# singer-yang/Aberration-Aware-Depth-from-Focus

Measured on NVIDIA B200. Metric: focal-stack Mpix*slices/s (fused PSFNet+PSF render), higher is better.
Workload: dtype fp16 hi/lo split, 3 terms for L1-L7, 2 terms on calibrated fp16 weights for L8, L9 and the head (worst case over any image 7.5e-5), f32 accumulate

## Files before the change

aberration-aware-depth-from-focus_b200/csrc/aadff_api.cu:

```cuda
#include <cuda_fp16.h>
#include <cuda_runtime.h>

#include <atomic>
#include <cmath>
#include <cstdio>
#include <cstring>
#include <mutex>
#include <string>
#include <vector>

#include "../../include/aadff.h"
#include "fused_tc_kernel.cuh"
#include "fused_fast2_kernel.cuh"
#include "gather_kernel.cuh"
#include "gather_coalesced_kernel.cuh"
#include "gather_strip_kernel.cuh"
#include "mlp_fp32_kernel.cuh"
#include "thinlens_kernel.cuh"
#include "focus_kernel.cuh"
#include "psf_conv_kernel.cuh"
#include "train_kernels.cuh"
#include "preprocess_kernel.cuh"
#include "spline_rotate_kernel.cuh"
#include "econ_calib.h"
// ... 432 lines not shown
        for (int l = 1; l < n_layers - 1; ++l, ++gi) {
            TcGroup& g = h->groups[gi];
            g.w_off = (uint32_t)(pack.size() * sizeof(__half));
            g.K = (uint16_t)dims[l];
            g.N = TC_HID;
            g.terms = 3;
            g.bias_off = (uint16_t)bias_tc.size();
            g.new_a = 1;
            g.tap0 = 0;
            pack_bias_slab(biases[l], TC_HID, pack);
            pack_group(weights[l], dims[l + 1], dims[l], 0, TC_HID, pack);
            bias_tc.insert(bias_tc.end(), biases[l], biases[l] + TC_HID);
        }
        h->n_hidden = gi;
        const int L = n_layers - 1;
        const int head_bias0 = (int)bias_tc.size();
        h->head_bias0 = head_bias0;
        bias_tc.resize(head_bias0 + nh_pad, 0.f);
        for (int n = 0; n < h->kk; ++n) bias_tc[head_bias0 + n] = -1.4426950408889634f * biases[L][n];
        for (int b = 0; b < n_head_blocks; ++b, ++gi) {
            TcGroup& g = h->groups[gi];
            const int N = std::min(256, nh_pad - 256 * b);
            g.w_off = (uint32_t)(pack.size() * sizeof(__half));
            g.K = TC_HID;
            g.N = (uint16_t)N;
            g.terms = 3;
            g.bias_off = (uint16_t)(head_bias0 + 256 * b);
            g.new_a = (b == 0);
            g.tap0 = (uint16_t)(256 * b);
            pack_group(weights[L], h->kk, TC_HID, 256 * b, N, pack);
        }
        h->n_groups = gi;
        h->n_bias = (int)bias_tc.size();
        h->host_dims.assign(dims, dims + n_layers + 1);
        for (int l = 0; l < n_layers; ++l) {
            h->host_w.emplace_back(weights[l], weights[l] + (size_t)dims[l] * dims[l + 1]);
            h->host_b.emplace_back(biases[l], biases[l] + dims[l + 1]);
        }
        h->pack_bytes = pack.size() * sizeof(__half);
        std::vector<float> w0b0(320);
        std::memcpy(w0b0.data(), weights[0], 256 * sizeof(float));
        std::memcpy(w0b0.data() + 256, biases[0], 64 * sizeof(float));
        __half* dp = nullptr;
        int rc = upload(pack, &dp);
        if (rc) { aadff_psfnet_destroy(h); return rc; }
        h->d_wpack = reinterpret_cast<uint8_t*>(dp);
        rc = upload(bias_tc, &h->d_bias_tc);
        if (rc) { aadff_psfnet_destroy(h); return rc; }
        rc = upload(w0b0, &h->d_w0b0);
        if (rc) { aadff_psfnet_destroy(h); return rc; }
        const int so = h->smem_optin;
        const auto attr = cudaFuncAttributeMaxDynamicSharedMemorySize;
        CREATE_TRY(cudaFuncSetAttribute(fused_psfnet_render_kernel<true, false, 0>, attr, so));
#define AADFF_SET_ATTR(U)                                                                        \
        CREATE_TRY(cudaFuncSetAttribute(fused_psfnet_render_kernel<false, false, U>, attr, so));   \
        CREATE_TRY(cudaFuncSetAttribute(fused_psfnet_render_kernel<false, false, U, true>, attr, so));   \
        CREATE_TRY(cudaFuncSetAttribute(fused_psfnet_render_kernel<false, true, U>, attr, so));
        AADFF_SET_ATTR(0) AADFF_SET_ATTR(1) AADFF_SET_ATTR(3) AADFF_SET_ATTR(13) AADFF_SET_ATTR(12) AADFF_SET_ATTR(15)
#undef AADFF_SET_ATTR
        CREATE_TRY(cudaFuncSetAttribute(fused_psfnet_render_kernel<false, false, 14>, attr, so));
        CREATE_TRY(cudaFuncSetAttribute(fused_psfnet_render_kernel<false, true, 14>, attr, so));
    }
#undef CREATE_TRY
    *out = h;
    return AADFF_OK;
}

int aadff_psfnet_destroy(aadff_psfnet_t h) {
    if (!h) return AADFF_OK;
    DeviceGuard guard(h->device);
    for (float* p : h->owned) cudaFree(p);
    cudaFree(h->d_wpack);
    cudaFree(h->d_wpack_econ);
    cudaFree(h->d_bias_tc);
    cudaFree(h->d_w0b0);
    cudaFree(h->ws);
    if (h->ws_stream) cudaStreamDestroy(h->ws_stream);
    if (h->ws_copy_stream) cudaStreamDestroy(h->ws_copy_stream);
    for (cudaEvent_t e : h->ws_events) cudaEventDestroy(e);
    delete h;
    return AADFF_OK;
}

static int ensure_econ(aadff_psfnet_t h) {
    std::lock_guard<std::mutex> lock(h->econ_mu);
    if (h->econ_ready) return AADFF_OK;
    const int n_layers = h->n_layers, L = n_layers - 1;
    std::vector<const float*> W(n_layers), B(n_layers);
    for (int l = 0; l < n_layers; ++l) { W[l] = h->host_w[l].data(); B[l] = h->host_b[l].data(); }
    std::vector<std::vector<float>> wq;
    calibrate_econ(W.data(), B.data(), h->host_dims.data(), n_layers, TC_ECON_FIRST_LAYER, wq);
    std::vector<__half> pack;
    for (int g2 = 0; g2 < h->n_groups; ++g2) {
        const bool hidden = g2 < h->n_hidden;
        const int l = hidden ? g2 + 1 : L;
        h->w_off_econ[g2] = h->groups[g2].w_off;
        if (l < TC_ECON_FIRST_LAYER || wq[l].empty()) continue;
        h->w_off_econ[g2] = (uint32_t)(h->pack_bytes + pack.size() * sizeof(__half));
        if (hidden) {
            pack_bias_slab(B[l], TC_HID, pack);
            pack_group(wq[l].data(), h->host_dims[l + 1], h->host_dims[l], 0, TC_HID, pack);
        } else {
            pack_group(wq[l].data(), h->kk, TC_HID, h->groups[g2].tap0, h->groups[g2].N, pack);
        }
    }
    uint8_t* d = nullptr;
    CUDA_TRY(cudaMalloc(reinterpret_cast<void**>(&d), h->pack_bytes + pack.size() * sizeof(__half)));
    cudaError_t e = cudaMemcpy(d, h->d_wpack, h->pack_bytes, cudaMemcpyDeviceToDevice);
    if (e == cudaSuccess) e = cudaMemcpy(d + h->pack_bytes, pack.data(), pack.size() * sizeof(__half), cudaMemcpyHostToDevice);
    if (e != cudaSuccess) {
        cudaFree(d);
        return fail(AADFF_E_CUDA, std::string("econ weight upload: ") + cudaGetErrorString(e));
    }
    h->d_wpack_econ = d;
// ... 89 lines not shown
        P.n_tiles = (tile_row1 - tile_row0) * P.tiles_x;
        if (P.n_tiles <= 0) return AADFF_OK;
    }
    if (probes != nullptr) {
        P.probes = probes;
        P.psf_out = psf_out;
        P.n_probes = n_probes;
        P.n_tiles = (n_probes + TC_M - 1) / TC_M;
    }
    P.trace = g_trace.load();
    P.dbg = (uint32_t)g_dbg_flags.load();
    uint32_t halo_bytes = (uint32_t)(TC_TILE_H + ra.ks - 1) * TC_HALO_PITCH * 16;
    if (probes != nullptr) halo_bytes = std::max<uint32_t>(halo_bytes, 8 * 32 * 9 * 4);
    const uint32_t bias_bytes = (uint32_t)(h->n_bias - h->head_bias0) * 4;
    const uint32_t ones_bytes = 2 * TC_A_LBO;
    const uint32_t bslab_bytes = 2 * TC_BSLAB_BYTES;
    const uint32_t fixed = 2 * TC_A_PART_BYTES + bias_bytes + 320 * 4 + halo_bytes + TC_M * 5 * 4 + TC_BAR_BYTES + ones_bytes +
                           bslab_bytes + 16;
    int stages = 4;
    while (stages >= 2 && fixed + (uint32_t)stages * TC_STAGE_BYTES > (uint32_t)h->smem_optin) --stages;
    if (stages < 2) return fail(AADFF_E_UNSUPPORTED, "shared memory budget exceeded for this kernel size / channel count");
    bool any_lo = false;
    for (int i = 0; i < h->n_groups; ++i) any_lo |= (P.g[i].terms >= 2);
    P.off_stage = 2 * TC_A_PART_BYTES;
    P.off_bias = P.off_stage + stages * TC_STAGE_BYTES;
    P.off_w0 = P.off_bias + bias_bytes;
    P.off_halo = P.off_w0 + 320 * 4;
    P.off_red = P.off_halo + halo_bytes;
    P.off_bar = P.off_red + TC_M * 5 * 4;
    P.off_ones = (P.off_bar + TC_BAR_BYTES + 15u) & ~15u;
    P.off_bslab = P.off_ones + ones_bytes;
    const uint32_t smem = P.off_bslab + bslab_bytes;
    P.kslab = (!any_lo && stages == 4) ? 2 : 1;
    P.n_stages = (P.kslab == 2) ? 4 : stages;
    int grid = (int)std::min<long long>(P.n_tiles, h->num_sms);
    bool all3 = true, all1 = true, econ_pat = true, econ8_pat = true, mixed_pat = true, aligned = (P.n_stages == 4 && P.kslab == 1);
    for (int i = 0; i < h->n_groups; ++i) {
        const int t = P.g[i].terms;
        all3 &= (t == 3);
        all1 &= (t == 1);
        econ_pat &= (t == (i < TC_ECON_FIRST_GROUP ? 3 : 2));
        econ8_pat &= (t == (i < TC_ECON8_FIRST_GROUP ? 3 : 2));
        mixed_pat &= (t == (i < TC_MIXED_FIRST_GROUP ? 3 : 1));
        aligned &= (((P.g[i].K / TC_SLAB_K) * (t == 3 ? 2 : 1)) % 4 == 0);
    }
    static_assert(TC_ECON_FIRST_GROUP == TC_ECON_FIRST_LAYER - 1, "group g holds layer g + 1");
    int uni = 0;
    if (all3 && P.kslab == 1) uni = aligned ? 13 : 3;
    else if (all1 && P.kslab == 2) uni = 1;
    else if (econ_pat && aligned) uni = 12;
    else if (econ8_pat && aligned && h->n_groups > TC_ECON8_FIRST_GROUP) uni = 14;
    else if (mixed_pat && aligned) uni = 15;
    const bool cl2 = P.probes == nullptr && P.trace == nullptr && uni != 0 && uni != 14 && (P.dbg & 8u) && h->num_sms >= 2;
    if (cl2) {
        grid = (int)std::min<long long>((P.n_tiles + 1) & ~1ll, (long long)(h->num_sms & ~1));
        cudaLaunchConfig_t cfg{};
        cfg.gridDim = dim3((unsigned)grid);
        cfg.blockDim = dim3(TC_NT);
        cfg.dynamicSmemBytes = smem;
        cfg.stream = st;
        cudaLaunchAttribute la[1];
        la[0].id = cudaLaunchAttributeClusterDimension;
        la[0].val.clusterDim.x = 2; la[0].val.clusterDim.y = 1; la[0].val.clusterDim.z = 1;
        cfg.attrs = la;
        cfg.numAttrs = 1;
        cudaError_t le = cudaSuccess;
        switch (uni) {
            case 1: le = cudaLaunchKernelEx(&cfg, fused_psfnet_render_kernel<false, false, 1, true>, P); break;
            case 3: le = cudaLaunchKernelEx(&cfg, fused_psfnet_render_kernel<false, false, 3, true>, P); break;
            case 13: le = cudaLaunchKernelEx(&cfg, fused_psfnet_render_kernel<false, false, 13, true>, P); break;
            case 12: le = cudaLaunchKernelEx(&cfg, fused_psfnet_render_kernel<false, false, 12, true>, P); break;
            default: le = cudaLaunchKernelEx(&cfg, fused_psfnet_render_kernel<false, false, 15, true>, P); break;
        }
        if (le != cudaSuccess) return fail(AADFF_E_CUDA, std::string("cluster launch: ") + cudaGetErrorString(le));
    } else if (P.trace != nullptr && P.probes == nullptr) {
        fused_psfnet_render_kernel<true, false, 0><<<grid, TC_NT, smem, st>>>(P);
    } else {
#define AADFF_LAUNCH(U)                                                                                   \
        case U:                                                                                           \
            if (P.probes != nullptr) fused_psfnet_render_kernel<false, true, U><<<grid, TC_NT, smem, st>>>(P);   \
            else fused_psfnet_render_kernel<false, false, U><<<grid, TC_NT, smem, st>>>(P);               \
            break;
        switch (uni) {
            AADFF_LAUNCH(1) AADFF_LAUNCH(3) AADFF_LAUNCH(13) AADFF_LAUNCH(12) AADFF_LAUNCH(14) AADFF_LAUNCH(15)
            default:
                if (P.probes != nullptr) fused_psfnet_render_kernel<false, true, 0><<<grid, TC_NT, smem, st>>>(P);
                else fused_psfnet_render_kernel<false, false, 0><<<grid, TC_NT, smem, st>>>(P);
        }
#undef AADFF_LAUNCH
    }
    g_launches.fetch_add(1);
    CUDA_TRY(cudaGetLastError());
    return AADFF_OK;
}

static int render_stack_impl(aadff_psfnet_t h, const float* img, const float* depth, const float* foc, int foc_stride,
                             float* out, const int64_t out_strides[5], int N, int C, int S, int H, int W, float d_min,
                             float d_max, int mode, void* stream, long long tile_row0 = 0, long long tile_row1 = -1);

int aadff_tile_row_height(void) { return TC_TILE_H; }
int aadff_econ_first_group(void) { return TC_ECON_FIRST_GROUP; }

int aadff_render_stack_rows_f32(aadff_psfnet_t h, const float* img, const float* depth, const float* foc, float* out,
                                const int64_t out_strides[5], int N, int C, int S, int H, int W, float d_min,
                                float d_max, int mode, int64_t tile_row_begin, int64_t tile_row_end, void* stream) {
    const long long total = (long long)N * S * ((H + TC_TILE_H - 1) / TC_TILE_H);
    if (tile_row_begin < 0 || tile_row_end < tile_row_begin || tile_row_end > total)
        return fail(AADFF_E_INVALID, "tile-row range outside [0, N*S*ceil(H/8)]");
    return render_stack_impl(h, img, depth, foc, S, out, out_strides, N, C, S, H, W, d_min, d_max, mode, stream,
                             tile_row_begin, tile_row_end);
}

int aadff_render_stack_f32(aadff_psfnet_t h, const float* img, const float* depth, const float* foc, float* out,
                           const int64_t out_strides[5], int N, int C, int S, int H, int W, float d_min,
                           float d_max, int mode, void* stream) {
    return render_stack_impl(h, img, depth, foc, S, out, out_strides, N, C, S, H, W, d_min, d_max, mode, stream);
}

static int render_stack_impl(aadff_psfnet_t h, const float* img, const float* depth, const float* foc, int foc_stride,
                             float* out, const int64_t out_strides[5], int N, int C, int S, int H, int W, float d_min,
                             float d_max, int mode, void* stream, long long tile_row0, long long tile_row1) {
    if (!h || !img || !depth || !foc || !out || !out_strides) return fail(AADFF_E_INVALID, "null argument");
    if (N < 0 || C < 1 || S < 1 || H < 1 || W < 1) return fail(AADFF_E_INVALID, "bad shape");
    if (mode < 0 || mode > 5) return fail(AADFF_E_INVALID, "unknown mode");
    if (d_max == d_min) return fail(AADFF_E_INVALID, "d_max == d_min");
    if (N == 0) return AADFF_OK;
    DeviceGuard guard(h->device);
    if (!guard.ok) return fail(AADFF_E_CUDA, "cannot select device");
    cudaStream_t st = static_cast<cudaStream_t>(stream);
    RenderArgs ra{};
    ra.img = img; ra.depth = depth; ra.foc = foc; ra.out = out;
    ra.os_n = out_strides[0]; ra.os_c = out_strides[1]; ra.os_s = out_strides[2];
    ra.os_h = out_strides[3]; ra.os_w = out_strides[4];
    ra.N = N; ra.S = S; ra.H = H; ra.W = W; ra.ks = h->ks; ra.Ctot = C;
    ra.foc_stride = foc_stride;
    ra.d_min = d_min;
    ra.d_range = d_max - d_min;
    ra.step_x = (W > 1) ? (1.0f - (-1.0f)) / (float)(W - 1) : 0.f;
    ra.step_y = (H > 1) ? (-1.0f - 1.0f) / (float)(H - 1) : 0.f;
    for (int c0 = 0; c0 < C; c0 += 4) {
        ra.c0 = c0;
        ra.C = std::min(4, C - c0);
// ... 544 lines not shown
```

aberration-aware-depth-from-focus_b200/csrc/fused_tc_kernel.cuh:

```cuda
#pragma once
#include <cuda_fp16.h>
#include <cuda_runtime.h>
#include "ptx_sm100.cuh"
#include "render_args.h"

namespace aadff {

constexpr int TC_TILE_H = 8;
constexpr int TC_TILE_W = 16;
constexpr int TC_M = TC_TILE_H * TC_TILE_W;
constexpr int TC_HALO_PITCH = 48;
constexpr int TC_HID = 256;
constexpr int TC_SLAB_K = 32;
constexpr int TC_STAGE_BYTES = TC_HID * TC_SLAB_K * 2;
constexpr int TC_A_PART_BYTES = TC_M * TC_HID * 2;
constexpr int TC_A_LBO = TC_M * 16;
constexpr int TC_EPI_WARPS = 8;
constexpr int TC_EPI_THREADS = TC_EPI_WARPS * 32;
constexpr int TC_NT = 64 + TC_EPI_THREADS;
constexpr int TC_MAX_GROUPS = 16;
constexpr int TC_MAX_STAGES = 8;
constexpr int TC_MAX_KS = 31;
constexpr int TC_MAX_C = 4;
constexpr int TC_BAR_BYTES = 256;
// ... 65 lines not shown
__device__ __forceinline__ uint32_t pack_half2_relu(float a, float b) {
    uint32_t r;
    asm("cvt.rn.relu.f16x2.f32 %0, %1, %2;" : "=r"(r) : "f"(b), "f"(a));
    return r;
}

__device__ __forceinline__ uint32_t pack_half2_relu_rz(float a, float b) {
    uint32_t r;
    asm("cvt.rz.relu.f16x2.f32 %0, %1, %2;" : "=r"(r) : "f"(b), "f"(a));
    return r;
}

__device__ __forceinline__ void store_split8(const float (&v)[8], uint32_t addr_hi, uint32_t addr_lo, bool need_lo) {
    uint32_t h[4];
#pragma unroll
    for (int u = 0; u < 4; ++u) h[u] = pack_half2(v[2 * u], v[2 * u + 1]);
    st_shared_v4(addr_hi, h[0], h[1], h[2], h[3]);
    if (need_lo) {
        uint32_t l[4];
#pragma unroll
        for (int u = 0; u < 4; ++u) {
            const float2 f = __half22float2(*reinterpret_cast<__half2*>(&h[u]));
            l[u] = pack_half2(v[2 * u] - f.x, v[2 * u + 1] - f.y);
        }
        st_shared_v4(addr_lo, l[0], l[1], l[2], l[3]);
    }
}

__device__ __forceinline__ void epi_group8(const uint32_t* acc, uint32_t a_hi, uint32_t a_lo,
                                           uint32_t kg, uint32_t a_row, bool need_lo) {
    if (!need_lo) {
        uint32_t h[4];
#pragma unroll
        for (int u = 0; u < 4; ++u) h[u] = pack_half2_relu(__uint_as_float(acc[2 * u]), __uint_as_float(acc[2 * u + 1]));
        st_shared_v4(a_hi + kg * TC_A_LBO + a_row, h[0], h[1], h[2], h[3]);
        return;
    }
    uint32_t h[4], l[4];
#pragma unroll
    for (int u = 0; u < 4; ++u) {
        const float a0 = __uint_as_float(acc[2 * u]), a1 = __uint_as_float(acc[2 * u + 1]);
        h[u] = pack_half2_relu_rz(a0, a1);
        const float2 f = __half22float2(*reinterpret_cast<__half2*>(&h[u]));
        l[u] = pack_half2_relu(a0 - f.x, a1 - f.y);
    }
    const uint32_t off = kg * TC_A_LBO + a_row;
    st_shared_v4(a_hi + off, h[0], h[1], h[2], h[3]);
    st_shared_v4(a_lo + off, l[0], l[1], l[2], l[3]);
}

constexpr int TC_WARP_PRODUCER = TC_EPI_WARPS;
constexpr int TC_WARP_MMA = TC_EPI_WARPS + 1;

template <bool TRACE, bool PRED, int UNI, bool CL2 = false>
__global__ void __launch_bounds__(TC_NT, 1) fused_psfnet_render_kernel(const __grid_constant__ TcParams P) {
    static_assert(!(CL2 && (PRED || TRACE)), "the cluster variant exists for the render kernels only");
    constexpr int UM = UNI % 10;
    const uint32_t cta_rank = CL2 ? cluster_ctarank() : 0u;
    const long long first_tile = CL2 ? (long long)(blockIdx.x & ~1u) : (long long)blockIdx.x;
    const long long my_iters = (P.n_tiles > first_tile) ? (P.n_tiles - first_tile + gridDim.x - 1) / gridDim.x : 0;
    constexpr bool ALIGNED = UNI >= 10;
    const int kslab_c = (UM == 3 || UM == 2 || UM == 4 || UM == 5) ? 1 : UM == 1 ? 2 : P.kslab;
    auto terms_of = [&](int gi) -> int {
        return UM == 3 ? 3 : UM == 1 ? 1 : UM == 2 ? (gi < TC_ECON_FIRST_GROUP ? 3 : 2)
                                         : UM == 4 ? (gi < TC_ECON8_FIRST_GROUP ? 3 : 2)
                                         : UM == 5 ? (gi < TC_MIXED_FIRST_GROUP ? 3 : 1) : (int)P.g[gi].terms;
    };
    extern __shared__ __align__(1024) uint8_t smem[];
    const uint32_t sbase = smem_u32(smem);
    const int warp = threadIdx.x >> 5, lane = threadIdx.x & 31;
    const RenderArgs& ra = P.ra;

    const uint32_t a_hi = sbase, a_lo = sbase + TC_A_PART_BYTES;
    const uint32_t stage0 = sbase + P.off_stage;
    const int stage_bytes = kslab_c * TC_STAGE_BYTES, stages_in_area = 4 / kslab_c;
    auto stage_addr = [&](int st) {
        return st < stages_in_area ? stage0 + st * stage_bytes : a_lo + (st - stages_in_area) * stage_bytes;
    };
    float* s_bias = reinterpret_cast<float*>(smem + P.off_bias);
    float* s_w0 = reinterpret_cast<float*>(smem + P.off_w0);
    float4* s_halo = reinterpret_cast<float4*>(smem + P.off_halo);
    float* s_red = reinterpret_cast<float*>(smem + P.off_red);
    const uint32_t bar0 = sbase + P.off_bar;
    auto bar_full = [&](int s) { return bar0 + 8u * s; };
    auto bar_empty = [&](int s) { return bar0 + 8u * (TC_MAX_STAGES + s); };
    auto bar_aready = [&](int j) { return bar0 + 8u * (2 * TC_MAX_STAGES + j); };
    auto bar_accfull = [&](int b) { return bar0 + 8u * (2 * TC_MAX_STAGES + 8 + b); };
    auto bar_accfree = [&](int b) { return bar0 + 8u * (2 * TC_MAX_STAGES + 10 + b); };
    auto bar_bfull = [&]() { return bar0 + 8u * (2 * TC_MAX_STAGES + 12); };
    auto bar_bempty = [&]() { return bar0 + 8u * (2 * TC_MAX_STAGES + 13); };
    volatile uint32_t* tmem_slot = reinterpret_cast<volatile uint32_t*>(smem + P.off_bar + 8 * (2 * TC_MAX_STAGES + 14));
    static_assert(8 * (2 * TC_MAX_STAGES + 14) + 4 <= TC_BAR_BYTES, "barrier area too small");

    if (threadIdx.x == 0) {
        for (int s = 0; s < TC_MAX_STAGES; ++s) { mbar_init(bar_full(s), 1); mbar_init(bar_empty(s), CL2 ? 2 : 1); }
        for (int j = 0; j < 8; ++j)
            mbar_init(bar_aready(j), (kslab_c == 2 || j < 4) ? TC_EPI_WARPS : 2 * TC_EPI_WARPS);
        for (int b = 0; b < 2; ++b) { mbar_init(bar_accfull(b), 1); mbar_init(bar_accfree(b), TC_EPI_WARPS); }
        mbar_init(bar_bfull(), 1);
        mbar_init(bar_bempty(), 1);
        fence_mbar_init();
    }
    for (int i = threadIdx.x; i < P.n_bias - P.bias_skip; i += TC_NT) s_bias[i] = __ldg(P.bias + P.bias_skip + i);
    for (int i = threadIdx.x; i < 2 * TC_M; i += TC_NT) {
        uint4 v = make_uint4(0u, 0u, 0u, 0u);
        if (i < TC_M) v.x = 0x3C003C00u;
        *reinterpret_cast<uint4*>(smem + P.off_ones + (i < TC_M ? 0 : TC_A_LBO) + (i % TC_M) * 16) = v;
    }
    for (int i = threadIdx.x; i < TC_BSLAB_BYTES / 16; i += TC_NT)
// ... 248 lines not shown
                if constexpr (PRED) {
                    const long long m = tile * TC_M + row;
                    nx_in = (m < P.n_probes) ? __ldg(reinterpret_cast<const float4*>(P.probes) + m)
                                             : make_float4(0.f, 0.f, 0.f, 0.f);
                } else {
                    int n, s, h0, w0;
                    tile_coords(tile, n, s, h0, w0);
                    const int hc = min(h0 + ty, ra.H - 1), wc = min(w0 + tx, ra.W - 1);
                    d = __ldg(ra.depth + ((long long)n * ra.H + hc) * ra.W + wc);
                    f = __ldg(ra.foc + (long long)n * ra.foc_stride + s);
                }
            }
        };
        float nx_depth = 0.f, nx_foc = 0.f;
        fetch_dz(blockIdx.x, nx_depth, nx_foc);

        auto layer0 = [&](long long t) {
            float x, y, z, fz;
            if constexpr (PRED) {
                x = nx_in.x; y = nx_in.y; z = nx_in.z; fz = nx_in.w;
            } else {
                int n, s, h0, w0;
                tile_coords(t, n, s, h0, w0);
                x = coord_x(min(w0 + tx, ra.W - 1), ra.W, ra.step_x);
                y = coord_y(min(h0 + ty, ra.H - 1), ra.H, ra.step_y);
                z = depth_to_z(nx_depth, ra.d_min, ra.d_range);
                fz = depth_to_z(nx_foc, ra.d_min, ra.d_range);
            }
            const bool need_lo = terms_of(0) >= 2;
#pragma unroll
            for (int i = 0; i < 4; ++i) {
                const int kg = fine ? ((i >> 1) * 4 + 2 * hh + (i & 1)) : (hh * 4 + i);
                float v[8];
#pragma unroll
                for (int u = 0; u < 8; ++u) {
                    const int f = kg * 8 + u;
                    const float4 wv = *reinterpret_cast<const float4*>(s_w0 + f * 4);
                    float a = s_w0[256 + f];
                    a = fmaf(wv.x, x, a); a = fmaf(wv.y, y, a); a = fmaf(wv.z, z, a); a = fmaf(wv.w, fz, a);
                    v[u] = fmaxf(a, 0.f);
                }
                const uint32_t off = (uint32_t)kg * TC_A_LBO + a_row;
                store_split8(v, a_hi + off, a_lo + off, need_lo);
            }
            fence_proxy_async_smem();
            __syncwarp();
            if (lane == 0) {
                if (fine) { mbar_arrive(bar_aready(0)); mbar_arrive(bar_aready(1)); }
                else mbar_arrive(bar_aready(0));
            }
        };
        if (my_iters > 0) layer0(blockIdx.x);

        long long tile = blockIdx.x;
        for (long long iter = 0; iter < my_iters; ++iter, tile += gridDim.x) {
            const bool dummy = CL2 && tile >= P.n_tiles;
            int n = 0, s = 0, h0 = 0, w0 = 0;
            if constexpr (!PRED) tile_coords(dummy ? 0 : tile, n, s, h0, w0);
            const int h = h0 + ty, w = w0 + tx;
            const long long m_row = tile * TC_M + row;
            const bool valid = PRED ? (m_row < P.n_probes) : ((h < ra.H) && (w < ra.W) && !dummy);
            tr.ev(0x800);
            fetch_dz(tile + gridDim.x, nx_depth, nx_foc);

            named_bar_sync(1, TC_EPI_THREADS);
            const float* img_n = ra.img + ((long long)n * ra.Ctot + ra.c0) * ra.H * ra.W;
            const long long cstride = (long long)ra.H * ra.W;
            auto halo_fetch = [&](int idx, float4& v) -> int {
                if (PRED || dummy || idx >= HH * HW) return -1;
                const int yy = idx / HW, xx = idx - yy * HW;
                const int gy = min(max(h0 + yy - r, 0), ra.H - 1), gx = min(max(w0 + xx - r, 0), ra.W - 1);
                const float* px = img_n + (long long)gy * ra.W + gx;
                v.x = __ldg(px);
                v.y = ra.C > 1 ? __ldg(px + cstride) : 0.f;
                v.z = ra.C > 2 ? __ldg(px + 2 * cstride) : 0.f;
                v.w = ra.C > 3 ? __ldg(px + 3 * cstride) : 0.f;
                return yy * TC_HALO_PITCH + xx;
            };

            for (int gi = 0; gi < P.n_hidden; ++gi) {
                const int buf = (int)(gcount & 1);
                float4 hv = make_float4(0.f, 0.f, 0.f, 0.f);
                const int hslot = halo_fetch(gi * TC_EPI_THREADS + et, hv);
                tr.ev(0xA00 + gi);
                mbar_wait(bar_accfull(buf), (afphase >> buf) & 1);
                afphase ^= 1u << buf;
                tc_fence_after_sync();
                tr.ev(0xB00 + gi);
                const bool need_lo = terms_of(gi + 1) >= 2;
                const uint32_t t_acc = t_lane + buf * 256;
                uint32_t rr[2][32], rf[2][16];
                if (fine) {
                    tmem_ld16(t_acc + hh * 16, rf[0]);
                    tmem_ld16(t_acc + 32 + hh * 16, rf[1]);
                } else {
                    tmem_ld32(t_acc + hh * 32, rr[0]);
                }
#pragma unroll
                for (int j = 0; j < 4; ++j) {
                    tmem_ld_wait();
                    if (j < 3) tmem_ld32(t_acc + (j + 1) * 64 + hh * 32, rr[(j + 1) & 1]);
                    if (j == 0 && fine) {
#pragma unroll
                        for (int c = 0; c < 2; ++c) {
                            const int col = c * 32 + hh * 16;
#pragma unroll
                            for (int i = 0; i < 2; ++i)
                                epi_group8(&rf[c][i * 8], a_hi, a_lo, col / 8 + i, a_row, need_lo);
                            fence_proxy_async_smem();
                            __syncwarp();
                            if (lane == 0) mbar_arrive(bar_aready(c));
                        }
                    } else {
                        const int col = j * 64 + hh * 32;
#pragma unroll
                        for (int i = 0; i < 4; ++i)
                            epi_group8(&rr[j & 1][i * 8], a_hi, a_lo, col / 8 + i, a_row, need_lo);
                        fence_proxy_async_smem();
                        __syncwarp();
                        if (lane == 0) mbar_arrive(bar_aready(fine ? (j == 1 ? 2 : 4) : j));
                    }
                    tr.ev(0xC00 + j);
                }
                tc_fence_before_sync();
                __syncwarp();
                if (lane == 0) mbar_arrive(bar_accfree(buf));
                if (hslot >= 0) s_halo[hslot] = hv;
                ++gcount;
            }
            for (int idx = P.n_hidden * TC_EPI_THREADS + et; !PRED && !dummy && idx < HH * HW; idx += TC_EPI_THREADS) {
                float4 hv;
                const int hslot = halo_fetch(idx, hv);
                s_halo[hslot] = hv;
            }
            named_bar_sync(1, TC_EPI_THREADS);

            float ssum = 0.f, cacc[TC_MAX_C] = {0.f, 0.f, 0.f, 0.f};
            const float4* hbase = s_halo + ty * TC_HALO_PITCH + tx;
            for (int gi = P.n_hidden; gi < P.n_groups; ++gi) {
                const int buf = (int)(gcount & 1);
                tr.ev(0xA00 + gi);
                mbar_wait(bar_accfull(buf), (afphase >> buf) & 1);
                afphase ^= 1u << buf;
                tc_fence_after_sync();
                tr.ev(0xB00 + gi);
                if (gi == P.n_groups - 1 && iter + 1 < my_iters) {
                    layer0(tile + gridDim.x);
                    tr.ev(0x900);
                }
                const int gN = P.g[gi].N, gtap0 = P.g[gi].tap0;
                const float* bias = s_bias + (P.g[gi].bias_off - P.bias_skip);
                if constexpr (PRED) {
                    if (pred_one_block) {
                        float keep[2][32];
#pragma unroll
                        for (int ci = 0; ci < 2; ++ci) {
                            const int c32 = hh * 32 + ci * 64;
                            if (c32 < gN) {
                                uint32_t rr[32];
                                tmem_ld32(t_lane + buf * 256 + c32, rr);
                                const int nvalid = kk - (gtap0 + c32);
                                tmem_ld_wait();
#pragma unroll
                                for (int u = 0; u < 32; ++u) {
                                    float sg = rcp_approx(1.0f + ex2_approx(fmaf(__uint_as_float(rr[u]), NEG_LOG2E, bias[c32 + u])));
                                    sg = (u < nvalid) ? sg : 0.f;
                                    keep[ci][u] = sg;
                                    ssum += sg;
                                }
                            } else {
#pragma unroll
                                for (int u = 0; u < 32; ++u) keep[ci][u] = 0.f;
                            }
                        }
                        tc_fence_before_sync();
                        __syncwarp();
                        if (lane == 0) mbar_arrive(bar_accfree(buf));
                        ++gcount;
                        s_red[row * 5 + hh] = ssum;
                        named_bar_sync(2 + q, 64);
                        const float inv = 1.0f / fmaxf(s_red[row * 5] + s_red[row * 5 + 1], 1e-12f);
                        float* stg = reinterpret_cast<float*>(s_halo) + e * (32 * 9);
                        const long long row0 = tile * TC_M + q * 32;
                        const int rsub = lane >> 3, csub = lane & 7;
#pragma unroll
                        for (int ci = 0; ci < 2; ++ci) {
#pragma unroll
                            for (int pc = 0; pc < 4; ++pc) {
                                const int c0 = gtap0 + hh * 32 + ci * 64 + pc * 8;
                                if (c0 >= kk) continue;
#pragma unroll
                                for (int j = 0; j < 8; ++j) stg[lane * 9 + j] = keep[ci][pc * 8 + j] * inv;
                                __syncwarp();
#pragma unroll
                                for (int rb = 0; rb < 8; ++rb) {
                                    const int rloc = rb * 4 + rsub;
                                    const float v = stg[rloc * 9 + csub];
                                    if (row0 + rloc < P.n_probes && c0 + csub < kk)
                                        P.psf_out[(row0 + rloc) * kk + c0 + csub] = v;
                                }
                                __syncwarp();
                            }
                        }
                        continue;
                    }
                }
#pragma unroll 1
                for (int c32 = hh * 32; c32 < gN; c32 += 64) {
                    uint32_t rr[32];
                    tmem_ld32(t_lane + buf * 256 + c32, rr);
                    const int tap_first = gtap0 + c32;
                    int i = tap_first / ks, j = tap_first - i * ks;
                    int off = i * TC_HALO_PITCH + j;
                    const int nvalid = kk - tap_first;
                    tmem_ld_wait();
                    if constexpr (PRED) {
                        float sgv[32];
#pragma unroll
                        for (int u = 0; u < 32; ++u) {
                            float sg = rcp_approx(1.0f + ex2_approx(fmaf(__uint_as_float(rr[u]), NEG_LOG2E, bias[c32 + u])));
                            sg = (u < nvalid) ? sg : 0.f;
                            sgv[u] = sg;
                            ssum += sg;
                        }
                        float* stg = reinterpret_cast<float*>(s_halo) + e * (32 * 9);
                        const long long row0 = tile * TC_M + q * 32;
                        const int rsub = lane >> 3, csub = lane & 7;
#pragma unroll
                        for (int pc = 0; pc < 4; ++pc) {
                            const int c0 = tap_first + pc * 8;
                            if (c0 >= kk) continue;
#pragma unroll
                            for (int j = 0; j < 8; ++j) stg[lane * 9 + j] = sgv[pc * 8 + j];
                            __syncwarp();
#pragma unroll
                            for (int rb = 0; rb < 8; ++rb) {
                                const int rloc = rb * 4 + rsub;
                                const float v = stg[rloc * 9 + csub];
                                if (row0 + rloc < P.n_probes && c0 + csub < kk) P.psf_out[(row0 + rloc) * kk + c0 + csub] = v;
                            }
                            __syncwarp();
                        }
                    } else if (nvalid >= 32) {
#pragma unroll
                        for (int u = 0; u < 32; ++u) {
                            const float sg = rcp_approx(1.0f + ex2_approx(fmaf(__uint_as_float(rr[u]), NEG_LOG2E, bias[c32 + u])));
                            const float4 px = hbase[off];
                            ssum += sg;
                            cacc[0] = fmaf(sg, px.x, cacc[0]);
                            cacc[1] = fmaf(sg, px.y, cacc[1]);
                            cacc[2] = fmaf(sg, px.z, cacc[2]);
                            cacc[3] = fmaf(sg, px.w, cacc[3]);
                            ++off;
                            if (++j == ks) { j = 0; off += TC_HALO_PITCH - ks; }
                        }
                    } else {
#pragma unroll
                        for (int u = 0; u < 32; ++u) {
                            const bool ok = u < nvalid;
                            float sg = rcp_approx(1.0f + ex2_approx(fmaf(__uint_as_float(rr[u]), NEG_LOG2E, bias[c32 + u])));
                            sg = ok ? sg : 0.f;
                            const float4 px = hbase[ok ? off : 0];
                            ssum += sg;
                            cacc[0] = fmaf(sg, px.x, cacc[0]);
                            cacc[1] = fmaf(sg, px.y, cacc[1]);
                            cacc[2] = fmaf(sg, px.z, cacc[2]);
                            cacc[3] = fmaf(sg, px.w, cacc[3]);
                            ++off;
                            if (++j == ks) { j = 0; off += TC_HALO_PITCH - ks; }
                        }
                    }
                }
                tc_fence_before_sync();
                __syncwarp();
                if (lane == 0) mbar_arrive(bar_accfree(buf));
                ++gcount;
            }
            if constexpr (PRED) {
                if (pred_one_block) continue;
                s_red[row * 5 + hh] = ssum;
                named_bar_sync(2 + q, 64);
                for (int rloc = hh * 16; rloc < hh * 16 + 16; ++rloc) {
                    const long long grow = tile * TC_M + q * 32 + rloc;
                    if (grow >= P.n_probes) break;
                    const float inv = 1.0f / fmaxf(s_red[(q * 32 + rloc) * 5] + s_red[(q * 32 + rloc) * 5 + 1], 1e-12f);
                    float* orow = P.psf_out + grow * kk;
                    for (int t = lane; t < kk; t += 32) orow[t] *= inv;
                }
                continue;
            }
            if (hh == 1) {
                s_red[row * 5 + 0] = ssum;
#pragma unroll
                for (int c = 0; c < TC_MAX_C; ++c) s_red[row * 5 + 1 + c] = cacc[c];
            }
            tr.ev(0xD00);
            named_bar_sync(2 + q, 64);
            if (hh == 0 && valid) {
                const float inv = 1.0f / fmaxf(ssum + s_red[row * 5], 1e-12f);
                float* o = ra.out + n * ra.os_n + ra.c0 * ra.os_c + s * ra.os_s + h * ra.os_h + w * ra.os_w;
#pragma unroll
                for (int c = 0; c < TC_MAX_C; ++c)
                    if (c < ra.C) o[c * ra.os_c] = (cacc[c] + s_red[row * 5 + 1 + c]) * inv;
            }
        }
    }

    tc_fence_before_sync();
    __syncthreads();
    if (CL2) cluster_sync_all();
    if (warp == TC_WARP_PRODUCER) tmem_dealloc<512>(tmem_base);
}

__global__ void __launch_bounds__(128, 1)
debug_umma_gemm_kernel(const float* __restrict__ A, const uint8_t* __restrict__ bpack, float* __restrict__ D,
                       int K, int N, uint32_t swap) {
    extern __shared__ __align__(1024) uint8_t smem[];
    const uint32_t sbase = smem_u32(smem);
    const int warp = threadIdx.x >> 5, lane = threadIdx.x & 31;
    const uint32_t a_hi = sbase;
    const uint32_t b_sm = sbase + TC_A_PART_BYTES;
    const uint32_t bar = sbase + TC_A_PART_BYTES + 131072;
    volatile uint32_t* slot = reinterpret_cast<volatile uint32_t*>(smem + TC_A_PART_BYTES + 131072 + 16);
    if (threadIdx.x == 0) { mbar_init(bar, 1); fence_mbar_init(); }
    if (warp == 0) tmem_alloc<256>(smem_u32(const_cast<uint32_t*>(slot)));
    const int row = threadIdx.x;
    for (int kg = 0; kg < K / 8; ++kg) {
        float v[8];
#pragma unroll
        for (int u = 0; u < 8; ++u) v[u] = A[(size_t)row * K + kg * 8 + u];
        store_split8(v, a_hi + kg * TC_A_LBO + row * 16, 0, false);
    }
    const int bbytes = (K / 32) * N * 64;
    for (int i = threadIdx.x * 16; i < bbytes; i += 128 * 16)
        *reinterpret_cast<uint4*>(smem + TC_A_PART_BYTES + i) = *reinterpret_cast<const uint4*>(bpack + i);
    fence_proxy_async_smem();
    tc_fence_before_sync();
    __syncthreads();
    tc_fence_after_sync();
    const uint32_t tmem_base = *slot;
    if (threadIdx.x == 0) {
        const uint32_t idesc = umma_idesc_f16_f32(128, N);
        const uint32_t lbo_b = (uint32_t)N * 16;
        for (int ks16 = 0; ks16 < K / 16; ++ks16) {
            const uint32_t slab = b_sm + (ks16 / 2) * (N * 64);
            umma_f16_ss(tmem_base, tc_desc(a_hi + ks16 * 2 * TC_A_LBO, TC_A_LBO, 128, swap),
                        tc_desc(slab + (ks16 & 1) * 2 * lbo_b, lbo_b, 128, swap), idesc, ks16 > 0);
        }
        umma_commit(bar);
    }
    __syncwarp();
    mbar_wait(bar, 0);
    tc_fence_after_sync();
    for (int c0 = 0; c0 < N; c0 += 32) {
        uint32_t rr[32];
        tmem_ld32(tmem_base + ((uint32_t)(warp * 32) << 16) + c0, rr);
        tmem_ld_wait();
// ... 110 lines not shown
```

Baseline: 484.7.

## Defer head-layer PSF gather into next tile's hidden-layer epilogue

Adds a DEFER kernel variant. It loads the head-layer accumulators into registers right away, frees the TMEM buffer, and launches the next tile's layer0 before doing any gather. The sigmoid-weighted halo gather and the output store for a tile then run during the next tile's hidden-layer epilogue slots (gi 0 and 1), so this work overlaps with tensor-core MMA instead of stalling the pipeline. The halo fetch is shifted two groups later to keep the previous tile's halo alive until it is consumed. This adds 64 registers of held raw values per thread plus extra named barriers, which risks register pressure and spills.

Measured after the change: 489.8, median of 6. Within noise of the previous version (+1.0%).

```diff
diff --git a/aberration-aware-depth-from-focus_b200/csrc/aadff_api.cu b/aberration-aware-depth-from-focus_b200/csrc/aadff_api.cu
--- a/aberration-aware-depth-from-focus_b200/csrc/aadff_api.cu
+++ b/aberration-aware-depth-from-focus_b200/csrc/aadff_api.cu
@@ -508,6 +508,7 @@
         const int so = h->smem_optin;
         const auto attr = cudaFuncAttributeMaxDynamicSharedMemorySize;
         CREATE_TRY(cudaFuncSetAttribute(fused_psfnet_render_kernel<true, false, 0>, attr, so));
+        CREATE_TRY(cudaFuncSetAttribute(fused_psfnet_render_kernel<true, false, 0, false, true>, attr, so));
 #define AADFF_SET_ATTR(U)                                                                        \
         CREATE_TRY(cudaFuncSetAttribute(fused_psfnet_render_kernel<false, false, U>, attr, so));   \
         CREATE_TRY(cudaFuncSetAttribute(fused_psfnet_render_kernel<false, false, U, true>, attr, so));   \
@@ -516,6 +517,9 @@
 #undef AADFF_SET_ATTR
         CREATE_TRY(cudaFuncSetAttribute(fused_psfnet_render_kernel<false, false, 14>, attr, so));
         CREATE_TRY(cudaFuncSetAttribute(fused_psfnet_render_kernel<false, true, 14>, attr, so));
+#define AADFF_SET_ATTR(U) CREATE_TRY(cudaFuncSetAttribute(fused_psfnet_render_kernel<false, false, U, false, true>, attr, so));
+        AADFF_SET_ATTR(0) AADFF_SET_ATTR(3) AADFF_SET_ATTR(13) AADFF_SET_ATTR(12) AADFF_SET_ATTR(14)
+#undef AADFF_SET_ATTR
     }
 #undef CREATE_TRY
     *out = h;
@@ -711,6 +715,8 @@
     else if (econ8_pat && aligned && h->n_groups > TC_ECON8_FIRST_GROUP) uni = 14;
     else if (mixed_pat && aligned) uni = 15;
     const bool cl2 = P.probes == nullptr && P.trace == nullptr && uni != 0 && uni != 14 && (P.dbg & 8u) && h->num_sms >= 2;
+    const bool defer = P.probes == nullptr && h->n_groups == h->n_hidden + 1 && h->groups[h->n_hidden].N <= 128 &&
+                       (uni == 0 || uni == 3 || uni == 13 || uni == 12 || uni == 14) && !(P.dbg & 4u);
     if (cl2) {
         grid = (int)std::min<long long>((P.n_tiles + 1) & ~1ll, (long long)(h->num_sms & ~1));
         cudaLaunchConfig_t cfg{};
@@ -733,20 +739,30 @@
         }
         if (le != cudaSuccess) return fail(AADFF_E_CUDA, std::string("cluster launch: ") + cudaGetErrorString(le));
     } else if (P.trace != nullptr && P.probes == nullptr) {
-        fused_psfnet_render_kernel<true, false, 0><<<grid, TC_NT, smem, st>>>(P);
+        if (defer) fused_psfnet_render_kernel<true, false, 0, false, true><<<grid, TC_NT, smem, st>>>(P);
+        else fused_psfnet_render_kernel<true, false, 0><<<grid, TC_NT, smem, st>>>(P);
     } else {
 #define AADFF_LAUNCH(U)                                                                                   \
         case U:                                                                                           \
             if (P.probes != nullptr) fused_psfnet_render_kernel<false, true, U><<<grid, TC_NT, smem, st>>>(P);   \
             else fused_psfnet_render_kernel<false, false, U><<<grid, TC_NT, smem, st>>>(P);               \
             break;
+#define AADFF_LAUNCH_DEFER(U)                                                                             \
+        case U:                                                                                           \
+            if (P.probes != nullptr) fused_psfnet_render_kernel<false, true, U><<<grid, TC_NT, smem, st>>>(P);   \
+            else if (defer) fused_psfnet_render_kernel<false, false, U, false, true><<<grid, TC_NT, smem, st>>>(P);   \
+            else fused_psfnet_render_kernel<false, false, U><<<grid, TC_NT, smem, st>>>(P);               \
+            break;
         switch (uni) {
-            AADFF_LAUNCH(1) AADFF_LAUNCH(3) AADFF_LAUNCH(13) AADFF_LAUNCH(12) AADFF_LAUNCH(14) AADFF_LAUNCH(15)
+            AADFF_LAUNCH(1) AADFF_LAUNCH(15)
+            AADFF_LAUNCH_DEFER(3) AADFF_LAUNCH_DEFER(13) AADFF_LAUNCH_DEFER(12) AADFF_LAUNCH_DEFER(14)
             default:
                 if (P.probes != nullptr) fused_psfnet_render_kernel<false, true, 0><<<grid, TC_NT, smem, st>>>(P);
+                else if (defer) fused_psfnet_render_kernel<false, false, 0, false, true><<<grid, TC_NT, smem, st>>>(P);
                 else fused_psfnet_render_kernel<false, false, 0><<<grid, TC_NT, smem, st>>>(P);
         }
 #undef AADFF_LAUNCH
+#undef AADFF_LAUNCH_DEFER
     }
     g_launches.fetch_add(1);
     CUDA_TRY(cudaGetLastError());
diff --git a/aberration-aware-depth-from-focus_b200/csrc/fused_tc_kernel.cuh b/aberration-aware-depth-from-focus_b200/csrc/fused_tc_kernel.cuh
--- a/aberration-aware-depth-from-focus_b200/csrc/fused_tc_kernel.cuh
+++ b/aberration-aware-depth-from-focus_b200/csrc/fused_tc_kernel.cuh
@@ -141,9 +141,10 @@
 constexpr int TC_WARP_PRODUCER = TC_EPI_WARPS;
 constexpr int TC_WARP_MMA = TC_EPI_WARPS + 1;
 
-template <bool TRACE, bool PRED, int UNI, bool CL2 = false>
+template <bool TRACE, bool PRED, int UNI, bool CL2 = false, bool DEFER = false>
 __global__ void __launch_bounds__(TC_NT, 1) fused_psfnet_render_kernel(const __grid_constant__ TcParams P) {
     static_assert(!(CL2 && (PRED || TRACE)), "the cluster variant exists for the render kernels only");
+    static_assert(!(DEFER && (PRED || CL2)), "the deferred gather exists for the one-CTA render kernels only");
     constexpr int UM = UNI % 10;
     const uint32_t cta_rank = CL2 ? cluster_ctarank() : 0u;
     const long long first_tile = CL2 ? (long long)(blockIdx.x & ~1u) : (long long)blockIdx.x;
@@ -498,6 +499,80 @@
         };
         if (my_iters > 0) layer0(blockIdx.x);
 
+        auto gather32 = [&](const uint32_t (&rr)[32], int gtap0, int c32, const float* bias, float& ssum,
+                            float (&cacc)[TC_MAX_C]) {
+            const float4* hbase = s_halo + ty * TC_HALO_PITCH + tx;
+            const int tap_first = gtap0 + c32;
+            int i = tap_first / ks, j = tap_first - i * ks;
+            int off = i * TC_HALO_PITCH + j;
+            const int nvalid = kk - tap_first;
+            if (nvalid >= 32) {
+#pragma unroll
+                for (int u = 0; u < 32; ++u) {
+                    const float sg = rcp_approx(1.0f + ex2_approx(fmaf(__uint_as_float(rr[u]), NEG_LOG2E, bias[c32 + u])));
+                    const float4 px = hbase[off];
+                    ssum += sg;
+                    cacc[0] = fmaf(sg, px.x, cacc[0]);
+                    cacc[1] = fmaf(sg, px.y, cacc[1]);
+                    cacc[2] = fmaf(sg, px.z, cacc[2]);
+                    cacc[3] = fmaf(sg, px.w, cacc[3]);
+                    ++off;
+                    if (++j == ks) { j = 0; off += TC_HALO_PITCH - ks; }
+                }
+            } else {
+#pragma unroll
+                for (int u = 0; u < 32; ++u) {
+                    const bool ok = u < nvalid;
+                    float sg = rcp_approx(1.0f + ex2_approx(fmaf(__uint_as_float(rr[u]), NEG_LOG2E, bias[c32 + u])));
+                    sg = ok ? sg : 0.f;
+                    const float4 px = hbase[ok ? off : 0];
+                    ssum += sg;
+                    cacc[0] = fmaf(sg, px.x, cacc[0]);
+                    cacc[1] = fmaf(sg, px.y, cacc[1]);
+                    cacc[2] = fmaf(sg, px.z, cacc[2]);
+                    cacc[3] = fmaf(sg, px.w, cacc[3]);
+                    ++off;
+                    if (++j == ks) { j = 0; off += TC_HALO_PITCH - ks; }
+                }
+            }
+        };
+        auto store_pixel = [&](float ssum, const float (&cacc)[TC_MAX_C], int n, int s, int h, int w, bool valid) {
+            if (hh == 1) {
+                s_red[row * 5 + 0] = ssum;
+#pragma unroll
+                for (int c = 0; c < TC_MAX_C; ++c) s_red[row * 5 + 1 + c] = cacc[c];
+            }
+            tr.ev(0xD00);
+            named_bar_sync(2 + q, 64);
+            if (hh == 0 && valid) {
+                const float inv = 1.0f / fmaxf(ssum + s_red[row * 5], 1e-12f);
+                float* o = ra.out + n * ra.os_n + ra.c0 * ra.os_c + s * ra.os_s + h * ra.os_h + w * ra.os_w;
+#pragma unroll
+                for (int c = 0; c < TC_MAX_C; ++c)
+                    if (c < ra.C) o[c * ra.os_c] = (cacc[c] + s_red[row * 5 + 1 + c]) * inv;
+            }
+        };
+        uint32_t hraw[2][32];
+        float pend_ssum = 0.f, pend_cacc[TC_MAX_C] = {0.f, 0.f, 0.f, 0.f};
+        auto deferred_half = [&](int ci, long long ptile) {
+            const TcGroup& hg = P.g[P.n_hidden];
+            if (ci == 0) {
+                pend_ssum = 0.f;
+#pragma unroll
+                for (int c = 0; c < TC_MAX_C; ++c) pend_cacc[c] = 0.f;
+            }
+            if (hh * 32 + ci * 64 < hg.N)
+                gather32(hraw[ci], hg.tap0, hh * 32 + ci * 64, s_bias + (hg.bias_off - P.bias_skip), pend_ssum, pend_cacc);
+            if (ci == 1) {
+                int n, s, h0, w0;
+                tile_coords(ptile, n, s, h0, w0);
+                const int h = h0 + ty, w = w0 + tx;
+                store_pixel(pend_ssum, pend_cacc, n, s, h, w, h < ra.H && w < ra.W);
+            }
+        };
+        const int gi_fin = min(1, P.n_hidden - 1);
+        constexpr int HALO_GI0 = DEFER ? 2 : 0;
+
         long long tile = blockIdx.x;
         for (long long iter = 0; iter < my_iters; ++iter, tile += gridDim.x) {
             const bool dummy = CL2 && tile >= P.n_tiles;
@@ -509,7 +584,7 @@
             tr.ev(0x800);
             fetch_dz(tile + gridDim.x, nx_depth, nx_foc);
 
-            named_bar_sync(1, TC_EPI_THREADS);
+            if (!DEFER) named_bar_sync(1, TC_EPI_THREADS);
             const float* img_n = ra.img + ((long long)n * ra.Ctot + ra.c0) * ra.H * ra.W;
             const long long cstride = (long long)ra.H * ra.W;
             auto halo_fetch = [&](int idx, float4& v) -> int {
@@ -527,7 +602,7 @@
             for (int gi = 0; gi < P.n_hidden; ++gi) {
                 const int buf = (int)(gcount & 1);
                 float4 hv = make_float4(0.f, 0.f, 0.f, 0.f);
-                const int hslot = halo_fetch(gi * TC_EPI_THREADS + et, hv);
+                const int hslot = gi >= HALO_GI0 ? halo_fetch((gi - HALO_GI0) * TC_EPI_THREADS + et, hv) : -1;
                 tr.ev(0xA00 + gi);
                 mbar_wait(bar_accfull(buf), (afphase >> buf) & 1);
                 afphase ^= 1u << buf;
@@ -571,18 +646,45 @@
                 tc_fence_before_sync();
                 __syncwarp();
                 if (lane == 0) mbar_arrive(bar_accfree(buf));
+                if (DEFER && iter > 0) {
+                    if (gi == 0) deferred_half(0, tile - gridDim.x);
+                    if (gi == gi_fin) {
+                        deferred_half(1, tile - gridDim.x);
+                        named_bar_sync(1, TC_EPI_THREADS);
+                    }
+                }
                 if (hslot >= 0) s_halo[hslot] = hv;
                 ++gcount;
             }
-            for (int idx = P.n_hidden * TC_EPI_THREADS + et; !PRED && !dummy && idx < HH * HW; idx += TC_EPI_THREADS) {
+            for (int idx = max(P.n_hidden - HALO_GI0, 0) * TC_EPI_THREADS + et; !PRED && !dummy && idx < HH * HW; idx += TC_EPI_THREADS) {
                 float4 hv;
                 const int hslot = halo_fetch(idx, hv);
                 s_halo[hslot] = hv;
             }
             named_bar_sync(1, TC_EPI_THREADS);
 
+            if constexpr (DEFER) {
+                const int gi = P.n_hidden, buf = (int)(gcount & 1);
+                tr.ev(0xA00 + gi);
+                mbar_wait(bar_accfull(buf), (afphase >> buf) & 1);
+                afphase ^= 1u << buf;
+                tc_fence_after_sync();
+                tr.ev(0xB00 + gi);
+#pragma unroll
+                for (int ci = 0; ci < 2; ++ci)
+                    if (hh * 32 + ci * 64 < P.g[gi].N) tmem_ld32(t_lane + buf * 256 + hh * 32 + ci * 64, hraw[ci]);
+                tmem_ld_wait();
+                tc_fence_before_sync();
+                __syncwarp();
+                if (lane == 0) mbar_arrive(bar_accfree(buf));
+                ++gcount;
+                if (iter + 1 < my_iters) {
+                    layer0(tile + gridDim.x);
+                    tr.ev(0x900);
+                }
+                continue;
+            }
             float ssum = 0.f, cacc[TC_MAX_C] = {0.f, 0.f, 0.f, 0.f};
-            const float4* hbase = s_halo + ty * TC_HALO_PITCH + tx;
             for (int gi = P.n_hidden; gi < P.n_groups; ++gi) {
                 const int buf = (int)(gcount & 1);
                 tr.ev(0xA00 + gi);
@@ -655,12 +757,10 @@
                 for (int c32 = hh * 32; c32 < gN; c32 += 64) {
                     uint32_t rr[32];
                     tmem_ld32(t_lane + buf * 256 + c32, rr);
-                    const int tap_first = gtap0 + c32;
-                    int i = tap_first / ks, j = tap_first - i * ks;
-                    int off = i * TC_HALO_PITCH + j;
-                    const int nvalid = kk - tap_first;
                     tmem_ld_wait();
                     if constexpr (PRED) {
+                        const int tap_first = gtap0 + c32;
+                        const int nvalid = kk - tap_first;
                         float sgv[32];
 #pragma unroll
                         for (int u = 0; u < 32; ++u) {
@@ -687,34 +787,8 @@
                             }
                             __syncwarp();
                         }
-                    } else if (nvalid >= 32) {
-#pragma unroll
-                        for (int u = 0; u < 32; ++u) {
-                            const float sg = rcp_approx(1.0f + ex2_approx(fmaf(__uint_as_float(rr[u]), NEG_LOG2E, bias[c32 + u])));
-                            const float4 px = hbase[off];
-                            ssum += sg;
-                            cacc[0] = fmaf(sg, px.x, cacc[0]);
-                            cacc[1] = fmaf(sg, px.y, cacc[1]);
-                            cacc[2] = fmaf(sg, px.z, cacc[2]);
-                            cacc[3] = fmaf(sg, px.w, cacc[3]);
-                            ++off;
-                            if (++j == ks) { j = 0; off += TC_HALO_PITCH - ks; }
-                        }
                     } else {
-#pragma unroll
-                        for (int u = 0; u < 32; ++u) {
-                            const bool ok = u < nvalid;
-                            float sg = rcp_approx(1.0f + ex2_approx(fmaf(__uint_as_float(rr[u]), NEG_LOG2E, bias[c32 + u])));
-                            sg = ok ? sg : 0.f;
-                            const float4 px = hbase[ok ? off : 0];
-                            ssum += sg;
-                            cacc[0] = fmaf(sg, px.x, cacc[0]);
-                            cacc[1] = fmaf(sg, px.y, cacc[1]);
-                            cacc[2] = fmaf(sg, px.z, cacc[2]);
-                            cacc[3] = fmaf(sg, px.w, cacc[3]);
-                            ++off;
-                            if (++j == ks) { j = 0; off += TC_HALO_PITCH - ks; }
-                        }
+                        gather32(rr, gtap0, c32, bias, ssum, cacc);
                     }
                 }
                 tc_fence_before_sync();
@@ -735,20 +809,12 @@
                 }
                 continue;
             }
-            if (hh == 1) {
-                s_red[row * 5 + 0] = ssum;
-#pragma unroll
-                for (int c = 0; c < TC_MAX_C; ++c) s_red[row * 5 + 1 + c] = cacc[c];
-            }
-            tr.ev(0xD00);
-            named_bar_sync(2 + q, 64);
-            if (hh == 0 && valid) {
-                const float inv = 1.0f / fmaxf(ssum + s_red[row * 5], 1e-12f);
-                float* o = ra.out + n * ra.os_n + ra.c0 * ra.os_c + s * ra.os_s + h * ra.os_h + w * ra.os_w;
-#pragma unroll
-                for (int c = 0; c < TC_MAX_C; ++c)
-                    if (c < ra.C) o[c * ra.os_c] = (cacc[c] + s_red[row * 5 + 1 + c]) * inv;
-            }
+            store_pixel(ssum, cacc, n, s, h, w, valid);
+        }
+        if (DEFER && my_iters > 0) {
+            const long long last = blockIdx.x + (my_iters - 1) * gridDim.x;
+            deferred_half(0, last);
+            deferred_half(1, last);
         }
     }
 
```
